# rvp-group/srrg2_slam_interfaces

Measured on AMD Instinct MI355X. Metric: icp_iterations_per_sec, higher is better.
Workload: dtype f32; 1 GPU; C2: SE(3) point-to-plane AlignerSlice, 100000-pt synthetic cloud pair per GPU, 10 ICP iterations per compute(), gated NN 0.25 m + normal gate, Cauchy 0.05; points=100000, alignments_total=1, all_success=True, last_status=0, last_num_inliers=99432, parallelism=single GPU

## Files before the change

### srrg2_slam_interfaces_amd/csrc/kernels.hip

```cpp
#include <climits>
#include <cstdlib>
#include <algorithm>

#include "kernels.h"
#include "search_plan.h"

#include <type_traits>

#include "det_math.h"

#include "device_util.h"

namespace {

#define FX_MAGIC 6755399441055744.0
#define FX_MAGIC_BITS 0x4338000000000000ll
__device__ __forceinline__ long long fx_bits(double biased) { return __double_as_longlong(biased) - FX_MAGIC_BITS; }

__device__ __forceinline__ unsigned long long key_min(unsigned long long a, unsigned long long b) {
  double r;
  asm("v_min_f64 %0, %1, %2" : "=v"(r) : "v"(__longlong_as_double((long long) a)), "v"(__longlong_as_double((long long) b)));
  return (unsigned long long) __double_as_longlong(r);
}

// ... 316 lines not shown
      local[threadIdx.x] += v;
    else if (v != 0)
      atomicAdd(reinterpret_cast<unsigned long long*>(partials) +
                  ((size_t) prob * PARTIAL_SLOTS + (block & (PARTIAL_SLOTS - 1))) * ACC_N + threadIdx.x,
                (unsigned long long) v);
  }
}

}

namespace {

struct QEntry {
  int i;
  int r2;
  float best;
  int bidx, bpos;
  float qx, qy, qz;
  float ball2;
  int pad_;
};
static_assert(sizeof(QEntry) == 40, "host reserves 10 words per entry");

__device__ __forceinline__ void finder_transform_of(const float* Sinv, int dim, const float* X, float* T) {
  if (dim == 3) {
    dm::se3_compose(Sinv, X, T);
  } else {
    float t9[9];
    dm::se2_compose(Sinv, X, t9);
    T[0] = t9[0]; T[1] = t9[1]; T[2] = 0.f; T[3] = t9[2];
    T[4] = t9[3]; T[5] = t9[4]; T[6] = 0.f; T[7] = t9[5];
    T[8] = 0.f; T[9] = 0.f; T[10] = 1.f; T[11] = 0.f;
  }
}
__device__ __forceinline__ void load_T(const float* src, float* T) {
#pragma unroll
  for (int i = 0; i < 12; ++i) T[i] = src[i];
}

template <int DIM>
__device__ __forceinline__ void transform_point(const float* T, const float4 p, float& qx, float& qy, float& qz) {
  if constexpr (DIM == 3) {
    qx = ((T[0] * p.x + T[1] * p.y) + T[2] * p.z) + T[3];
    qy = ((T[4] * p.x + T[5] * p.y) + T[6] * p.z) + T[7];
    qz = ((T[8] * p.x + T[9] * p.y) + T[10] * p.z) + T[11];
  } else {
    qx = (T[0] * p.x + T[1] * p.y) + T[3];
    qy = (T[4] * p.x + T[5] * p.y) + T[7];
    qz = 0.f;
  }
}

constexpr int STAGE_CAP = 64;
template <int DIM, int TW, bool STAGE = false>
__device__ __forceinline__ void coop_scan(const GridDev& g, int lane, int* lds_wave, float sqx, float sqy, float sqz,
                                          int scx, int scy, int scz, int sr, float sr2, float& wbest, int& widx,
                                          int& wpos, float& wexcl2, float4* stage = nullptr) {
  constexpr int ROWS_PER_CHUNK = 2 * TW;
  const int lt   = lane & (TW - 1);
  const int team = lane / TW;
  int* flat      = lds_wave + team * (4 * TW + 8);
  int* first     = flat + ROWS_PER_CHUNK + 4;
  const float rr = ball_radius(sr2);
  int x0, x1, y0, y1, z0 = 0, z1 = 0;
  axis_range(sqx, rr, g.ox, g.inv_h, scx - sr, scx + sr, g.nx, x0, x1);
  axis_range(sqy, rr, g.oy, g.inv_h, scy - sr, scy + sr, g.ny, y0, y1);
  if (DIM == 3) axis_range(sqz, rr, g.oz, g.inv_h, scz - sr, scz + sr, g.nz, z0, z1);
  auto row_range = [&](int rrow, int ny_r, int& rs, int& re) {
    const int y = y0 + rrow % ny_r, z = z0 + rrow / ny_r;
    const float ylo = g.oy + (float) y * g.h;
    float dy        = fmaxf(fmaxf(ylo - sqy, sqy - (ylo + g.h)), 0.f);
    dy              = fmaxf(dy - (0.01f * g.h + (fabsf(sqy) + rr) * 2e-6f), 0.f);
    float rem       = rr * rr - dy * dy;
    if (DIM == 3) {
      const float zlo = g.oz + (float) z * g.h;
      float dz        = fmaxf(fmaxf(zlo - sqz, sqz - (zlo + g.h)), 0.f);
      dz              = fmaxf(dz - (0.01f * g.h + (fabsf(sqz) + rr) * 2e-6f), 0.f);
      rem             = rem - dz * dz;
    }
    rs = re = 0;
    if (!(rem < 0.f)) {
      int xa = x0, xb = x1;
      if (rem < 3.0e38f) axis_range(sqx, ball_radius(rem), g.ox, g.inv_h, x0, x1, g.nx, xa, xb);
      if (xa <= xb) {
        const int row = (z * g.ny + y) * g.nx;
        rs = g.cell_start[row + xa];
        re = g.cell_start[row + xb + 1];
      }
    }
  };
  unsigned long long key = NO_KEY;
  float lb2              = INFINITY;
  const bool any = sr >= 0 && x0 <= x1 && y0 <= y1 && z0 <= z1;
  const int ny_r = any ? y1 - y0 + 1 : 1;
  const int rows = any ? ny_r * (z1 - z0 + 1) : 0;
  int max_rows = rows;
  if (TW < 64) {
#pragma unroll
    for (int off = TW; off < 64; off <<= 1) max_rows = max(max_rows, __shfl_xor(max_rows, off));
  }
  [[maybe_unused]] int staged = 0;
  for (int row0 = 0; row0 < max_rows; row0 += ROWS_PER_CHUNK) {
    int sA = 0, eA = 0, sB = 0, eB = 0;
    const int rA = row0 + lt, rB = row0 + TW + lt;
    if (rA < rows) row_range(rA, ny_r, sA, eA);
    if (rB < rows) row_range(rB, ny_r, sB, eB);
    const unsigned long long pk = (unsigned long long) (unsigned) (eA - sA) | ((unsigned long long) (unsigned) (eB - sB) << 32);
    unsigned long long inc = pk;
#pragma unroll
    for (int off = 1; off < TW; off <<= 1) {
      unsigned long long t = __shfl_up(inc, off, TW);
      if (lt >= off) inc += t;
    }
    const unsigned long long tot = __shfl(inc, TW - 1, TW);
    const int totA = (int) (unsigned) tot, totB = (int) (tot >> 32);
    const unsigned long long exc = inc - pk;
    flat[lt]       = (int) (unsigned) exc;
    flat[TW + lt]  = totA + (int) (exc >> 32);
    first[lt]      = sA;
    first[TW + lt] = sB;
    if (lt == 0) flat[ROWS_PER_CHUNK] = totA + totB;
    wave_lds_sync();
    const int total = totA + totB;
    const int share = (total + TW - 1) / TW;
    int t           = lt * share;
    const int tend  = min(t + share, total);
    if (t < tend) {
      int lo = 0, hi = ROWS_PER_CHUNK - 1;
#pragma unroll
      for (int it = 0; it < 7; ++it) {
        if ((1 << it) >= ROWS_PER_CHUNK) break;
        const int mid = (lo + hi + 1) >> 1;
        if (flat[mid] <= t) lo = mid; else hi = mid - 1;
      }
      int r    = lo;
      int next = flat[r + 1];
      while (t < tend) {
        while (t >= next) {
          ++r;
          next = flat[r + 1];
        }
        const int j   = first[r] + (t - flat[r]);
        const int run = min(next, tend) - t;
        if constexpr (STAGE) {
          if (staged + total <= STAGE_CAP)
            for (int c = 0; c < run; ++c) stage[staged + t + c] = g.pts[j + c];
        } else {
          scan_range2<DIM>(g.pts, j, j + run, sqx, sqy, sqz, key, lb2);
        }
        t += run;
      }
    }
    if constexpr (STAGE) staged += total;
    wave_lds_sync();
  }
  if constexpr (STAGE) {
    wbest = INFINITY; widx = staged; wpos = 0; wexcl2 = 0.f;
    return;
  }
  unsigned long long kmin = key;
#pragma unroll
  for (int off = TW / 2; off >= 1; off >>= 1) {
    const unsigned long long o = __shfl_xor(kmin, off);
    kmin = o < kmin ? o : kmin;
  }
  wpos  = 0;
  wbest = __uint_as_float((unsigned) (kmin >> 32));
  widx  = (int) (unsigned) kmin;
  float v = key == kmin ? lb2 : fminf(lb2, __uint_as_float((unsigned) (key >> 32)));
#pragma unroll
  for (int off = TW / 2; off >= 1; off >>= 1) v = fminf(v, __shfl_xor(v, off));
  wexcl2 = fminf(v, fminf(sr2, bound2_of(max(sr, 0), g.h)));
}

namespace {

#ifndef SRRG2_CNL_REDEAL
#define SRRG2_CNL_REDEAL 0
#endif
#ifdef SRRG2_CNL_STATS
__device__ unsigned long long g_cnl_stats[4 * 16];
#define CNL_STAT(k, v)                                                                                   \
  do {                                                                                                   \
    const unsigned long long v_ = (unsigned long long) (v);    \
    if ((threadIdx.x & 63) == 0) atomicAdd(&g_cnl_stats[(stat_it < 3 ? stat_it : 3) * 16 + (k)], v_);    \
  } while (0)
#else
#define CNL_STAT(k, v) do { } while (0)
#endif
constexpr int CNL_POOL = 512;

struct CnlWave {
  uint2 pool[CNL_POOL];
  unsigned long long key[64];
  unsigned b2[64];
  float q[3][64];
};

template <int DIM>
// ... 1204 lines not shown
      float wbest, wexcl2;
      int widx, wpos;
      coop_scan<DIM, 64>(g, lane, wlds[wid].coop, __shfl(qx, src), __shfl(qy, src), __shfl(qz, src), __shfl(cx, src),
                         __shfl(cy, src), __shfl(cz, src), __shfl(r2, src), __shfl(ball2, src), wbest, widx, wpos, wexcl2);
      if (lane == src) excl_wide = sqrtf(wexcl2) * 0.99999f;
      if (lane == src && (wbest < best || (wbest == best && widx < bidx))) {
        best = wbest;
        bidx = widx;
      }
      continue;
    }
    int src[4];
#pragma unroll
    for (int t = 0; t < 4; ++t) {
      src[t] = need ? __ffsll((long long) need) - 1 : -1;
      need &= need - 1;
    }
    const int team = lane >> 4;
    const int mine = team == 0 ? src[0] : (team == 1 ? src[1] : (team == 2 ? src[2] : src[3]));
    const int from = mine >= 0 ? mine : lane;
    float wbest, wexcl2;
    int widx, wpos;
    const int sr_from = __shfl(r2, from);
    coop_scan<DIM, 16>(g, lane, wlds[wid].coop, __shfl(qx, from), __shfl(qy, from), __shfl(qz, from), __shfl(cx, from),
                       __shfl(cy, from), __shfl(cz, from), mine >= 0 ? sr_from : -1, __shfl(ball2, from), wbest, widx, wpos,
                       wexcl2);
#pragma unroll
    for (int t = 0; t < 4; ++t) {
      const float rb = __shfl(wbest, 16 * t), re = __shfl(wexcl2, 16 * t);
      const int ri = __shfl(widx, 16 * t);
      if (lane == src[t]) {
        excl_wide = sqrtf(re) * 0.99999f;
        if (rb < best || (rb == best && ri < bidx)) {
          best = rb;
          bidx = ri;
        }
      }
    }
  }
  if (excl_wide != 0.f || r2 != 0) excl = excl_wide;
  long long acc[ACC_N];
#pragma unroll
  for (int a = 0; a < ACC_N; ++a) acc[a] = 0;
  finish_point<DIM, PLANE>(S, T, rk, thr, kk, scale, inrange, active, gi, oi, p, qx, qy, qz, best, bidx, bpos, excl, skipped,
                           pf, pn, pnm, use_prior && S.use_normal_gate, acc);
  block_reduce_store<NW>(acc, S.partials, prob, tile, nullptr);
}

#ifdef SRRG2_PASS_TIMELINE
#define PASS_TS_WGS 2048
__device__ unsigned long long g_pass_ts[16 * PASS_TS_WGS * 8];
#define PASS_TS_ANY(epoch, k)                       \
  do {                                                                                                 \
    if ((threadIdx.x & 63) == 0 && (epoch) >= 0 && (epoch) < 16 && blockIdx.y < PASS_TS_WGS - 2 && blockIdx.x == 0) \
      g_pass_ts[(((epoch) * PASS_TS_WGS) + blockIdx.y) * 8 + (k)] = wall_clock64();                            \
  } while (0)
#define PASS_TS_W(epoch, k, dep)              \
  do {                                                                                                 \
    if (threadIdx.x == 0 && (epoch) >= 0 && (epoch) < 16 && blockIdx.x == 0) {                         \
      unsigned long long t_ = wall_clock64();                                                          \
      if ((dep) != (dep)) t_ = 0;         \
      g_pass_ts[(((epoch) * PASS_TS_WGS) + 0) * 8 + (k)] = t_;                                                  \
    }                                                                                                  \
  } while (0)
#define PASS_TS(epoch, k)                                                                              \
  do {                                                                                                 \
    if (threadIdx.x == 0 && (epoch) >= 0 && (epoch) < 16 && blockIdx.y < PASS_TS_WGS - 2 && blockIdx.x == 0)       \
      g_pass_ts[(((epoch) * PASS_TS_WGS) + blockIdx.y) * 8 + (k)] = wall_clock64();                            \
  } while (0)
#else
#define PASS_TS(epoch, k) do { } while (0)
#define PASS_TS_ANY(epoch, k) do { } while (0)
#define PASS_TS_W(epoch, k, dep) do { } while (0)
#endif
namespace {

__device__ float robust_weight(int kind, float thr, float chi, bool& kernelized);
template <bool PAIRS = false, bool GIVEN = true>
__device__ __forceinline__ int slice_exponent(const CtlParams& C, const SliceCtl& s, int prob, int nm, const float* T,
                                              int* kh_out = nullptr);
template <bool ONLY_INLINE, bool PAIRS = false>
__device__ __forceinline__ void init_problem_thread0(const CtlParams& C, int prob, const ProblemDev* probs_host, ProblemDev* probs,
                                                     ProblemState* states, const float* guesses_host, int tsize,
                                                     const InitInline& inl, unsigned (*init_gran)[PUB_SLICE_GRANULES]);

__device__ __forceinline__ double rl_d(double v, int k) {
  const int lo = __builtin_amdgcn_readlane(__double2loint(v), k);
  const int hi = __builtin_amdgcn_readlane(__double2hiint(v), k);
  return __hiloint2double(hi, lo);
}
__device__ __forceinline__ long long rl_ll(long long v, int k) {
  const int lo = __builtin_amdgcn_readlane((int) (unsigned) v, k);
  const int hi = __builtin_amdgcn_readlane((int) (unsigned) ((unsigned long long) v >> 32), k);
  return (long long) (((unsigned long long) (unsigned) hi << 32) | (unsigned) lo);
}
__device__ __forceinline__ float rl_f(float v, int k) { return __int_as_float(__builtin_amdgcn_readlane(__float_as_int(v), k)); }
__device__ __forceinline__ double wave_max_d(double v) {
#pragma unroll
  for (int off = 32; off >= 1; off >>= 1) {
    const double o = __shfl_xor(v, off);
    v              = o > v ? o : v;
  }
  return v;
}
__device__ __forceinline__ double wave_min_d(double v) {
#pragma unroll
  for (int off = 32; off >= 1; off >>= 1) {
    const double o = __shfl_xor(v, off);
    v              = o < v ? o : v;
  }
  return v;
}

__device__ __forceinline__ unsigned long long pub_load(const unsigned long long* p) {
  return __hip_atomic_load(p, __ATOMIC_RELAXED, __HIP_MEMORY_SCOPE_AGENT);
}
__device__ __forceinline__ void pub_store(unsigned long long* p, unsigned long long v) {
  __hip_atomic_store(p, v, __ATOMIC_RELAXED, __HIP_MEMORY_SCOPE_AGENT);
}

// ... 481 lines not shown

struct PassView {
  float T[12], Tprev[12];
  int kexp;
  bool stop, phase1, prior;
};

__device__ __forceinline__ void pass_view_legacy(const SliceDev& S, const ProblemState* __restrict__ st, PassView& v) {
#pragma unroll
  for (int i = 0; i < 12; ++i) v.T[i] = st->Tf[S.slice_idx][i];
#pragma unroll
  for (int i = 0; i < 12; ++i) v.Tprev[i] = st->Tfprev[S.slice_idx][i];
  v.kexp   = st->kexp[S.slice_idx];
  v.stop   = st->done || st->finished;
  v.phase1 = st->phase == 1;
  v.prior  = st->nstats > 0 || st->phase == 1;
}

#ifndef SRRG2_FUSED_POLL_LIMIT
#define SRRG2_FUSED_POLL_LIMIT 64
#endif
#ifdef SRRG2_FUSED_STALL
__device__ unsigned long long g_fused_fallbacks;
extern "C" int srrg2_amd_debug_fused_fallbacks(unsigned long long* out, int reset) {
  if (out && hipMemcpyFromSymbol(out, HIP_SYMBOL(g_fused_fallbacks), sizeof(unsigned long long)) != hipSuccess) return -1;
  if (reset) {
    const unsigned long long zero = 0;
    if (hipMemcpyToSymbol(HIP_SYMBOL(g_fused_fallbacks), &zero, sizeof(zero)) != hipSuccess) return -1;
  }
  return 0;
}
#define FUSED_STALL()                                                              \
  do {                                                                             \
    for (int stall_i = 0; stall_i < (SRRG2_FUSED_STALL); ++stall_i) __builtin_amdgcn_s_sleep(127); \
  } while (0)
#define FUSED_FALLBACK_COUNT()                                                     \
  do {                                                                             \
    if ((threadIdx.x & 63) == 0) atomicAdd(&g_fused_fallbacks, 1ull);              \
  } while (0)
__device__ unsigned long long g_stage_counts[6];
extern "C" int srrg2_amd_debug_staged_neighbours(unsigned long long* out6, int reset) {
  if (out6 && hipMemcpyFromSymbol(out6, HIP_SYMBOL(g_stage_counts), 6 * sizeof(unsigned long long)) != hipSuccess) return -1;
  if (reset) {
    const unsigned long long zero[6] = {0, 0, 0, 0, 0, 0};
    if (hipMemcpyToSymbol(HIP_SYMBOL(g_stage_counts), zero, sizeof(zero)) != hipSuccess) return -1;
  }
  return 0;
}
#define STAGE_COUNT(k, n)                                   \
  do {                                                                             \
    const unsigned long long n_ = (unsigned long long) (n);                        \
    if ((threadIdx.x & 63) == 0 && n_) atomicAdd(&g_stage_counts[k], n_);          \
  } while (0)
#else
#define FUSED_STALL() do { } while (0)
#define FUSED_FALLBACK_COUNT() do { } while (0)
#ifdef SRRG2_PASS_TIMELINE
#define STAGE_COUNT(k, n)                                                                                        \
  do {                                                                                                           \
    const unsigned long long n_ = (unsigned long long) (n);                                                      \
    if ((threadIdx.x & 63) == 0 && n_ && S.fc.epoch >= 0 && S.fc.epoch < 16 && blockIdx.x == 0)                  \
      atomicAdd(&g_pass_ts[((size_t) S.fc.epoch * PASS_TS_WGS + PASS_TS_WGS - 2) * 8 + (k)], n_);                \
  } while (0)
#else
#define STAGE_COUNT(k, n) do { } while (0)
#endif
#endif
#ifndef STAGE_THIN_A
#define STAGE_THIN_A 2.0f
#endif
#ifndef STAGE_THIN_B
#define STAGE_THIN_B 1e-5f
#endif

template <int DIM, bool PRIORS = false>
__device__ __forceinline__ void fused_control_if_due(const SliceDev& S, ProblemState* __restrict__ states, int prob) {
  if (blockIdx.y != 0 || threadIdx.x >= 64) return;
  const unsigned long long g[1] = {
    pub_load(S.fc.pub + ((size_t) prob * SRRG2_MAX_SLICES + S.slice_idx) * PUB_SLICE_GRANULES + (threadIdx.x & 63))};
  if (!__all((unsigned) (g[0] >> 32) == (unsigned) S.fc.epoch)) {
    FUSED_STALL();
    wave_control<DIM == 3 ? 6 : 3, 1, true, PRIORS>(&S, 1, states, prob, g);
  }
  PASS_TS(S.fc.epoch, 1);
}

struct NoStaging {};
template <int DIM, bool PRIORS = false, class WhileWaiting = NoStaging>
__device__ __forceinline__ void pass_view_fused(const SliceDev& S, ProblemState* __restrict__ states, int prob, PassView& v,
                                                WhileWaiting while_waiting = WhileWaiting{}) {
  constexpr bool STAGING = !std::is_same<WhileWaiting, NoStaging>::value;
  __shared__ unsigned rec_lds[PUB_SLICE_GRANULES];
  [[maybe_unused]] __shared__ unsigned stale_lds[STAGING ? 25 : 1];
  const int lane = threadIdx.x & 63;
  [[maybe_unused]] unsigned long long g_first = 0;
  if constexpr (STAGING) {
    if (threadIdx.x < 64) {
      const unsigned long long* rec = S.fc.pub + ((size_t) prob * SRRG2_MAX_SLICES + S.slice_idx) * PUB_SLICE_GRANULES + lane;
      const bool late = (int) (blockIdx.y * gridDim.x + blockIdx.x) >= S.fc.first_round;
      g_first         = late ? *rec : pub_load(rec);
      const bool whole_prev = __all((unsigned) (g_first >> 32) == (unsigned) (S.fc.epoch - 1));
      if (lane < 24) stale_lds[lane] = (unsigned) g_first;
      if (lane == 24) stale_lds[24] = whole_prev ? 1u : 0u;
    }
    __syncthreads();
    while_waiting(stale_lds);
  }
  if (threadIdx.x < 64) {
    const unsigned long long* rec = S.fc.pub + ((size_t) prob * SRRG2_MAX_SLICES + S.slice_idx) * PUB_SLICE_GRANULES + lane;
    const bool late      = (int) (blockIdx.y * gridDim.x + blockIdx.x) >= S.fc.first_round;
    unsigned long long g;
    if constexpr (STAGING) g = g_first; else g = late ? *rec : pub_load(rec);
    if (!__all((unsigned) (g >> 32) == (unsigned) S.fc.epoch)) {
      const unsigned* ep = S.fc.pub_epoch + ((size_t) prob * PUB_EPOCH_REPLICAS + (blockIdx.y & (PUB_EPOCH_REPLICAS - 1))) * PUB_EPOCH_STRIDE;
      int spins = 0;
      for (;;) {
        if ((int) __hip_atomic_load(ep, __ATOMIC_RELAXED, __HIP_MEMORY_SCOPE_AGENT) >= S.fc.epoch) {
          g = pub_load(rec);
// ... 457 lines not shown
      }
    }
#pragma unroll
    for (int r = 0; r < ROWS; ++r) {
      J[r][0] = m[r][0];
      J[r][1] = m[r][1];
      J[r][2] = m[r][1] * p.x - m[r][0] * p.y;
    }
  }
}

}

template <int DIM, bool PLANE, int PPT, bool GATHER, int FUSED>
__device__ __forceinline__ void icp_step_fast_body(const SliceDev& S, const ProblemDev* __restrict__ probs,
                                                   ProblemState* __restrict__ states) {
  constexpr int D    = DIM == 3 ? 6 : 3;
  constexpr int ROWS = PLANE ? 1 : DIM;
  const int prob     = (FUSED ? blockIdx.x : blockIdx.y) + S.prob0;
  const int tile     = FUSED ? (int) blockIdx.y : (int) blockIdx.x;
  const ProblemState* st = &states[prob];
  PassView pv;
  if constexpr (!FUSED) {
    pass_view_legacy(S, st, pv);
    if (pv.stop) return;
  } else {
    PASS_TS(S.fc.epoch, 0);
    fused_control_if_due<DIM, FUSED == 2>(S, states, prob);
  }
  const ProblemDev pd = probs[prob];
  if (tile * (256 * PPT) >= pd.nm && (!FUSED || tile != 0)) return;
  float T[12], Tprev[12];
  double scale;
  int rk;
  if constexpr (!FUSED) {
    load_T(pv.T, T);
    load_T(pv.Tprev, Tprev);
    scale = dm::pow2(pv.kexp);
    rk    = (pv.phase1 && S.robust_kind != SRRG2_ROBUST_NONE) ? (int) SRRG2_ROBUST_CLAMP : S.robust_kind;
  }
  const float thr    = S.robust_thr;
  const float kk     = S.variable_kind == SRRG2_SE3_QUAT_RIGHT ? 2.f : 1.f;
  const GridDev& g   = S.grid;
  const float gfar   = g.gate2_ext;
  const int rfar     = g.rmax;
  const float gate_r = S.gate * 1.000001f;
  const bool ngate   = S.use_normal_gate != 0;
  const bool use_q   = !FUSED && S.queue != nullptr && st->qmode[S.slice_idx] != 0;
  const int lane     = threadIdx.x & 63;
  const int wid      = threadIdx.x >> 6;
  struct StageWave {
    int coop[288];
    float4 cand[4][STAGE_CAP];
  };
  union FastWaveLds {
    CnlWave cnl;
    int coop[288];
    StageWave stage;
  };
  static_assert(sizeof(StageWave) <= sizeof(CnlWave), "the staged candidates live in the idle pool of the list search");
  __shared__ FastWaveLds fast_lds[4];
  int* const coop_lds_w = fast_lds[wid].coop;

  auto linearize = [&](auto first, long long (&acc)[ACC_N], bool valid, const float4 pk, const float4 fk, const float4 nk,
                       const float4 nmk, float qx, float qy, float qz, float best) {
    bool found = valid && __float_as_int(fk.w) != NO_MATCH && best <= g.gate2;
    if (ngate) {
      float dot;
      if constexpr (DIM == 3) {
        const float rx = (T[0] * nmk.x + T[1] * nmk.y) + T[2] * nmk.z;
        const float ry = (T[4] * nmk.x + T[5] * nmk.y) + T[6] * nmk.z;
        const float rz = (T[8] * nmk.x + T[9] * nmk.y) + T[10] * nmk.z;
        dot            = (nk.x * rx + nk.y * ry) + nk.z * rz;
      } else {
        const float rx = T[0] * nmk.x + T[1] * nmk.y;
        const float ry = T[4] * nmk.x + T[5] * nmk.y;
        dot            = nk.x * rx + nk.y * ry;
      }
      found = found && dot > S.normal_cos;
    }
    float J[ROWS][D], e[ROWS];
    point_rows<DIM, PLANE>(T, kk, pk, qx, qy, qz, fk, nk, J, e);
    (void) factor_accumulate_flat<D, ROWS, decltype(first)::value>(J, e, found, rk, thr, scale, acc);
  };

  long long acc[ACC_N];

  float4 p[PPT], pf[PPT], pnm[PPT], pn[PPT];
  float pm[PPT];
  int gi_[PPT];
  bool inr[PPT];
#pragma unroll
  for (int k = 0; k < PPT; ++k) {
    const int i = (tile * PPT + k) * 256 + (int) threadIdx.x;
    inr[k]      = i < pd.nm;
    gi_[k]      = pd.moff + (inr[k] ? i : 0);
    int ppos    = -1;
    p[k]        = S.mpts[gi_[k]];
    pm[k]       = S.prev_m[gi_[k]];
    pf[k]       = make_float4(0.f, 0.f, 0.f, __int_as_float(NO_MATCH));
    pn[k]       = make_float4(0.f, 0.f, 0.f, 0.f);
    pnm[k]      = make_float4(0.f, 0.f, 0.f, 0.f);
    if (GATHER) {
      ppos = S.prev_pos[gi_[k]];
    } else {
      pf[k] = S.prev_f[gi_[k]];
      if (PLANE || ngate) pn[k] = S.prev_n[gi_[k]];
    }
    if (ngate) pnm[k] = S.mnrm[gi_[k]];
    if (GATHER && ppos >= 0 && ppos < g.n) {
      pf[k] = g.pts[ppos];
      if (PLANE || ngate) pn[k] = g.nrm[ppos];
    }
  }
  constexpr bool STAGE = PPT == 1 && FUSED == 1 && !GATHER;
  [[maybe_unused]] unsigned long long st_mask = 0;
  [[maybe_unused]] int st_n = 0;
  [[maybe_unused]] float st_R2 = 0.f;
  [[maybe_unused]] float Tst[12];
  [[maybe_unused]] auto stage_thin = [&](const unsigned* stale) {
    if (!__builtin_amdgcn_readfirstlane((int) stale[24])) return;
    float Tpp[12];
#pragma unroll
    for (int i = 0; i < 12; ++i) Tst[i] = __int_as_float(__builtin_amdgcn_readfirstlane((int) stale[i]));
#pragma unroll
    for (int i = 0; i < 12; ++i) Tpp[i] = __int_as_float(__builtin_amdgcn_readfirstlane((int) stale[12 + i]));
    float ax, ay, az, bx, by, bz;
    transform_point<DIM>(Tst, p[0], ax, ay, az);
    transform_point<DIM>(Tpp, p[0], bx, by, bz);
    const float ex = ax - bx, ey = ay - by, ez = az - bz;
    const float dlp = __builtin_amdgcn_sqrtf((ex * ex + ey * ey) + ez * ez);
    unsigned long long k0 = NO_KEY;
    test_candidate<DIM>(pf[0], ax, ay, az, true, k0);
    const float d0 = __builtin_amdgcn_sqrtf(key_best(k0));
    const float rr = (d0 + PAD_MIN * g.h) * 1.00001f;
    const float R2 = fminf(rr * rr, gfar);
    const bool thin = inr[0] && finite3(p[0].x, p[0].y, p[0].z) && __float_as_int(pf[0].w) != NO_MATCH &&
                      R2 <= bound2_of(2, g.h) && pm[0] * 0.99999f - d0 * 1.00001f < STAGE_THIN_A * dlp + STAGE_THIN_B * g.h;
    unsigned long long m = __ballot(thin);
    const int nthin      = __popcll(m);
    if (nthin == 0) return;
    if (nthin > 4) {
      STAGE_COUNT(5, 1);
      return;
    }
    st_mask = m;
    st_R2   = R2;
    int src[4];
#pragma unroll
    for (int t = 0; t < 4; ++t) {
      src[t] = m ? __ffsll((long long) m) - 1 : -1;
      m &= m - 1;
    }
    const int team = lane >> 4;
    const int mine = team == 0 ? src[0] : (team == 1 ? src[1] : (team == 2 ? src[2] : src[3]));
    const int from = mine >= 0 ? mine : lane;
    const float sqx = __shfl(ax, from), sqy = __shfl(ay, from), sqz = __shfl(az, from), sball = __shfl(R2, from);
    const int scx = cell_coord(sqx, g.ox, g.inv_h), scy = cell_coord(sqy, g.oy, g.inv_h);
    const int scz = DIM == 3 ? cell_coord(sqz, g.oz, g.inv_h) : 0;
    float wbest, wexcl2;
    int wpos, count;
    coop_scan<DIM, 16, true>(g, lane, fast_lds[wid].stage.coop, sqx, sqy, sqz, scx, scy, scz, mine >= 0 ? 2 : -1, sball, wbest,
                             count, wpos, wexcl2, fast_lds[wid].stage.cand[team]);
    st_n = mine >= 0 ? count : 0;
    STAGE_COUNT(0, nthin);
    PASS_TS_ANY(S.fc.epoch, 5);
  };
  if constexpr (FUSED) {
    if constexpr (STAGE)
      pass_view_fused<DIM, false>(S, states, prob, pv, stage_thin);
    else
      pass_view_fused<DIM, FUSED == 2>(S, states, prob, pv);
    if (pv.stop || tile * (256 * PPT) >= pd.nm) return;
    load_T(pv.T, T);
    load_T(pv.Tprev, Tprev);
    scale = dm::pow2(pv.kexp);
    rk    = (pv.phase1 && S.robust_kind != SRRG2_ROBUST_NONE) ? (int) SRRG2_ROBUST_CLAMP : S.robust_kind;
  }

  float open_ball2[PPT];
  bool any_open = false;
  auto search_open = [&](float (&sbest)[PPT], int (&sidx)[PPT], float (&sexcl)[PPT], int (&spos)[PPT]) {
  #pragma unroll
    for (int k = 0; k < PPT; ++k) {
      sbest[k] = INFINITY; sexcl[k] = 0.f; sidx[k] = NO_MATCH; spos[k] = 0;
      bool open = open_ball2[k] >= 0.f;
      if (!__ballot(open)) continue;
      float qx = 0.f, qy = 0.f, qz = 0.f;
      if (open) transform_point<DIM>(T, p[k], qx, qy, qz);
      if constexpr (STAGE) {
        const unsigned long long due = st_mask & __ballot(open);
        STAGE_COUNT(4, __popcll(__ballot(open) & ~st_mask));
        if (due) {
          int src[4];
          unsigned long long m = st_mask;
#pragma unroll
          for (int t = 0; t < 4; ++t) {
            src[t] = m ? __ffsll((long long) m) - 1 : -1;
            m &= m - 1;
          }
          const int team = lane >> 4, lt = lane & 15;
          const int mine = team == 0 ? src[0] : (team == 1 ? src[1] : (team == 2 ? src[2] : src[3]));
          const int from = mine >= 0 ? mine : lane;
          const float sqx = __shfl(qx, from), sqy = __shfl(qy, from), sqz = __shfl(qz, from);
          const bool work = mine >= 0 && ((due >> (mine & 63)) & 1ull) && st_n <= STAGE_CAP;
          unsigned long long key = NO_KEY;
          float lb2 = INFINITY;
          if (work) {
            const float4* cand = fast_lds[wid].stage.cand[team];
            for (int c = lt; c < st_n; c += 16) test_candidate2<DIM>(cand[c], sqx, sqy, sqz, true, key, lb2);
          }
          unsigned long long kmin = key;
#pragma unroll
          for (int off = 8; off >= 1; off >>= 1) {
            const unsigned long long o = __shfl_xor(kmin, off);
            kmin = o < kmin ? o : kmin;
          }
          float v = key == kmin ? lb2 : fminf(lb2, key_best(key));
#pragma unroll
          for (int off = 8; off >= 1; off >>= 1) v = fminf(v, __shfl_xor(v, off));
          bool decided = false, overflow = false;
#pragma unroll
          for (int t = 0; t < 4; ++t) {
            const unsigned long long rk_ = __shfl(kmin, 16 * t);
            const float rv = __shfl(v, 16 * t);
            const int rn   = __shfl(st_n, 16 * t);
            if (lane == src[t] && open) {
              float ax, ay, az;
              transform_point<DIM>(Tst, p[k], ax, ay, az);
              const float ex = qx - ax, ey = qy - ay, ez = qz - az;
              const float dls = sqrtf((ex * ex + ey * ey) + ez * ez);
              const float rin = sqrtf(st_R2) * 0.99999f - dls * 1.00001f;
              overflow = rn > STAGE_CAP;
              if (!overflow && key_idx(rk_) != NO_MATCH && sqrtf(key_best(rk_)) * 1.00001f < rin) {
                sbest[k] = key_best(rk_);
                sidx[k]  = key_idx(rk_);
                sexcl[k] = sqrtf(fminf(rv, rin * rin)) * 0.99999f;
                decided  = true;
              }
            }
          }
          STAGE_COUNT(1, __popcll(__ballot(decided)));
          STAGE_COUNT(2, __popcll(__ballot(overflow)));
          STAGE_COUNT(3, __popcll(due) - __popcll(__ballot(decided || overflow)));
          open = open && !decided;
          if (!__ballot(open)) continue;
        }
      }
      if (g.list_R > 0 && __popcll(__ballot(open)) > 4) {
        unsigned long long skey;
        float sb2, sL;
        cnl_search<DIM, 1>(g, *g.lists, fast_lds[wid].cnl, lane, open, qx, qy, qz, open_ball2[k], gfar, skey, sb2, sL);
        if (open) {
          sbest[k] = key_best(skey);
          sidx[k]  = key_idx(skey);
          sexcl[k] = sqrtf(fminf(sb2, fminf(sL, g.gate2_ext))) * 0.99999f;
        }
        continue;
      }
      bool open_k = open;
      if constexpr (PPT == 1) {
        if (!(g.list_R > 0) && __popcll(__ballot(open)) > 4) {
          unsigned long long lkey = NO_KEY;
          float lb2 = INFINITY, lc2 = INFINITY;
          if (open)
            scan_radius1<DIM>(g, qx, qy, qz, cell_coord(qx, g.ox, g.inv_h), cell_coord(qy, g.oy, g.inv_h),
                              DIM == 3 ? cell_coord(qz, g.oz, g.inv_h) : 0, open_ball2[k], lkey, lb2, lc2);
          const float b2_1 = bound2_of(1, g.h);
          if (open && key_idx(lkey) != NO_MATCH && key_best(lkey) <= gfar && key_best(lkey) <= b2_1) {
            sbest[k] = key_best(lkey);
            sidx[k]  = key_idx(lkey);
            sexcl[k] = sqrtf(fminf(fminf(lb2, lc2), b2_1)) * 0.99999f;
            open_k   = false;
          }
        }
      }
      const int r2 = open_ball2[k] <= bound2_of(2, g.h) ? 2 : max(rfar, 3);
      unsigned long long near = __ballot(open_k && r2 == 2);
      while (near) {
        int src[4];
  #pragma unroll
        for (int t = 0; t < 4; ++t) {
          src[t] = near ? __ffsll((long long) near) - 1 : -1;
          near &= near - 1;
        }
        const int team = lane >> 4;
        const int mine = team == 0 ? src[0] : (team == 1 ? src[1] : (team == 2 ? src[2] : src[3]));
        const int from = mine >= 0 ? mine : lane;
        const float sqx = __shfl(qx, from), sqy = __shfl(qy, from), sqz = __shfl(qz, from), sball = __shfl(open_ball2[k], from);
        const int scx = cell_coord(sqx, g.ox, g.inv_h), scy = cell_coord(sqy, g.oy, g.inv_h);
        const int scz = DIM == 3 ? cell_coord(sqz, g.oz, g.inv_h) : 0;
// ... 34 lines not shown
  };
  constexpr bool defer = PPT == 1 && FUSED;
  float d_qx = 0.f, d_qy = 0.f, d_qz = 0.f, d_best = INFINITY;
  bool d_valid = false;
#pragma unroll
  for (int k = 0; k < PPT; ++k) {
    const bool active = inr[k] && finite3(p[k].x, p[k].y, p[k].z);
    float qx, qy, qz, px, py, pz;
    transform_point<DIM>(T, p[k], qx, qy, qz);
    transform_point<DIM>(Tprev, p[k], px, py, pz);
    const float ex = qx - px, ey = qy - py, ez = qz - pz;
    const float dl   = __builtin_amdgcn_sqrtf((ex * ex + ey * ey) + ez * ez);
    const bool hasp  = __float_as_int(pf[k].w) != NO_MATCH;
    unsigned long long k1 = NO_KEY;
    test_candidate<DIM>(pf[k], qx, qy, qz, true, k1);
    const float best = key_best(k1);
    const float d1   = __builtin_amdgcn_sqrtf(best);
    const float rhs  = pm[k] * 0.99999f;
    const bool ca   = hasp && (d1 * 1.00001f + dl * 1.00001f < rhs);
    const bool cc   = !hasp && pm[k] > 0.f && (gate_r * 1.00001f + dl * 1.00001f < rhs);
    const bool have = active && (ca || cc);
    const float excl = pm[k] * 0.9999999f - dl * 1.00001f;
    const float pad  = fminf(2.f * dl, PAD_CAP * g.h) + PAD_MIN * g.h;
    const float rr   = (d1 + pad) * 1.00001f;
    const float r2box = hasp ? fminf(rr * rr, gfar) : gfar;
    open_ball2[k]     = (active && !have) ? r2box : -1.f;
    any_open |= active && !have;
#ifdef SRRG2_PASS_TIMELINE
    if constexpr (FUSED) {
      if (active && !have && S.fc.epoch >= 0 && S.fc.epoch < 16 && blockIdx.x == 0) {
        unsigned long long* c = &g_pass_ts[((size_t) S.fc.epoch * PASS_TS_WGS + PASS_TS_WGS - 1) * 8];
        const float gap = (pm[k] - d1) / g.h;
        atomicAdd(&c[0], 1ull);
        if (!hasp) atomicAdd(&c[1], 1ull);
        else if (gap < 1e-4f) atomicAdd(&c[2], 1ull);
        else if (gap < 0.0202f) atomicAdd(&c[3], 1ull);
        else atomicAdd(&c[4], 1ull);
        if (dl > 1e-3f * g.h) atomicAdd(&c[5], 1ull);
        if (pm[k] <= 0.f) atomicAdd(&c[6], 1ull);
      }
    }
#endif
    if constexpr (defer) {
      d_qx = qx; d_qy = qy; d_qz = qz; d_best = best; d_valid = have && ca;
    } else if (k == 0) {
      linearize(std::true_type{}, acc, have && ca, p[k], pf[k], pn[k], pnm[k], qx, qy, qz, best);
    } else {
      linearize(std::false_type{}, acc, have && ca, p[k], pf[k], pn[k], pnm[k], qx, qy, qz, best);
    }
    if (have) S.prev_m[gi_[k]] = excl;
  }
  if constexpr (defer) {
    {
      if (__any(any_open)) {
        float sbest[PPT], sexcl[PPT];
        int sidx[PPT], spos[PPT];
        search_open(sbest, sidx, sexcl, spos);
        const bool open = open_ball2[0] >= 0.f;
        const bool same = open && sidx[0] != NO_MATCH && sidx[0] == __float_as_int(pf[0].w);
        if (open && !same) {
          pf[0] = make_float4(0.f, 0.f, 0.f, __int_as_float(NO_MATCH));
          pn[0] = make_float4(0.f, 0.f, 0.f, 0.f);
          if (sidx[0] != NO_MATCH) {
            spos[0] = g.pos_of[sidx[0]];
            pf[0]   = g.pts[spos[0]];
            if (PLANE || ngate) pn[0] = g.nrm[spos[0]];
          }
          S.prev_pos[gi_[0]] = sidx[0] != NO_MATCH ? spos[0] : -1;
          if (!GATHER) {
            S.prev_f[gi_[0]] = pf[0];
            if (PLANE || ngate) S.prev_n[gi_[0]] = pn[0];
          }
        }
        if (open) {
          S.prev_m[gi_[0]] = sexcl[0];
          d_best  = sbest[0];
          d_valid = true;
        }
      }
      linearize(std::true_type{}, acc, d_valid, p[0], pf[0], pn[0], pnm[0], d_qx, d_qy, d_qz, d_best);
      block_reduce_store_biased<4>(acc, S.partials, prob, tile, PPT);
      if constexpr (FUSED) PASS_TS(S.fc.epoch, 3);
      return;
    }
  }
  if (use_q) {
#pragma unroll
    for (int k = 0; k < PPT; ++k) {
      const bool open               = open_ball2[k] >= 0.f;
      const unsigned long long need = __ballot(open);
      if (!need) continue;
      const int r2 = open_ball2[k] <= bound2_of(2, g.h) ? 2 : max(rfar, 3);
      const unsigned long long need_near = __ballot(open && r2 == 2);
      const unsigned long long need_far  = need & ~need_near;
      int base_near = 0, base_far = 0;
      if (lane == 0) {
        if (need_near) base_near = atomicAdd(&S.qcount[2 * prob], __popcll(need_near));
        if (need_far) base_far = atomicAdd(&S.qcount[2 * prob + 1], __popcll(need_far));
      }
      base_near = __shfl(base_near, 0);
      base_far  = __shfl(base_far, 0);
      if (open) {
        const unsigned long long below = (1ull << lane) - 1ull;
        QEntry q;
        q.i = (tile * PPT + k) * 256 + (int) threadIdx.x;
        q.r2 = r2; q.best = INFINITY; q.bidx = NO_MATCH; q.bpos = 0;
        transform_point<DIM>(T, p[k], q.qx, q.qy, q.qz);
        q.ball2 = open_ball2[k]; q.pad_ = 0;
        QEntry* qbase = reinterpret_cast<QEntry*>(S.queue) + pd.moff;
        if (r2 == 2)
          qbase[base_near + __popcll(need_near & below)] = q;
        else
          qbase[pd.nm - 1 - (base_far + __popcll(need_far & below))] = q;
      }
    }
  }
  block_reduce_store_biased<4, 1>(acc, S.partials, prob, tile, PPT);
  if (use_q || !__any(any_open)) {
    block_reduce_store_biased<4, 2>(acc, S.partials, prob, tile, PPT);
    if constexpr (FUSED) PASS_TS(S.fc.epoch, 3);
    return;
  }

  float sbest[PPT], sexcl[PPT];
  int sidx[PPT], spos[PPT];
  search_open(sbest, sidx, sexcl, spos);
  long long acc2[ACC_N];
#pragma unroll
  for (int k = 0; k < PPT; ++k) {
    const bool open = open_ball2[k] >= 0.f;
    float4 fk = make_float4(0.f, 0.f, 0.f, __int_as_float(NO_MATCH)), nk = make_float4(0.f, 0.f, 0.f, 0.f);
    bool same = false;
    if constexpr (PPT == 1) same = open && sidx[k] != NO_MATCH && sidx[k] == __float_as_int(pf[k].w);
    if (same) {
// ... 2227 lines not shown
```

Measured before the change: 65140 iterations/s.

## Add per-query near-candidate fast path and thin-lane fallback in staged NN search

Result: faster. 66310 iterations/s, median of 6 (+1.8%).

```diff
diff --git a/srrg2_slam_interfaces_amd/csrc/kernels.hip b/srrg2_slam_interfaces_amd/csrc/kernels.hip
--- a/srrg2_slam_interfaces_amd/csrc/kernels.hip
+++ b/srrg2_slam_interfaces_amd/csrc/kernels.hip
@@ -392,10 +392,15 @@
 }
 
 constexpr int STAGE_CAP = 64;
+constexpr int STAGE_NEAR = 5;
+struct StageNear {
+  int n[4];
+  float4 f[4][STAGE_NEAR];
+};
 template <int DIM, int TW, bool STAGE = false>
 __device__ __forceinline__ void coop_scan(const GridDev& g, int lane, int* lds_wave, float sqx, float sqy, float sqz,
                                           int scx, int scy, int scz, int sr, float sr2, float& wbest, int& widx,
-                                          int& wpos, float& wexcl2, float4* stage = nullptr) {
+                                          int& wpos, float& wexcl2, float4* stage = nullptr, StageNear* near = nullptr) {
   constexpr int ROWS_PER_CHUNK = 2 * TW;
   const int lt   = lane & (TW - 1);
   const int team = lane / TW;
@@ -484,7 +489,14 @@
         const int run = min(next, tend) - t;
         if constexpr (STAGE) {
           if (staged + total <= STAGE_CAP)
-            for (int c = 0; c < run; ++c) stage[staged + t + c] = g.pts[j + c];
+            for (int c = 0; c < run; ++c) {
+              const float4 f        = g.pts[j + c];
+              stage[staged + t + c] = f;
+              if (!(cand_d2<DIM>(f, sqx, sqy, sqz) > sr2 * 1.000001f)) {
+                const int at = atomicAdd(&near->n[team], 1);
+                if (at < STAGE_NEAR) near->f[team][at] = f;
+              }
+            }
         } else {
           scan_range2<DIM>(g.pts, j, j + run, sqx, sqy, sqz, key, lb2);
         }
@@ -1795,7 +1807,7 @@
 __device__ unsigned long long g_pass_ts[16 * PASS_TS_WGS * 8];
 #define PASS_TS_ANY(epoch, k)                       \
   do {                                                                                                 \
-    if ((threadIdx.x & 63) == 0 && (epoch) >= 0 && (epoch) < 16 && blockIdx.y < PASS_TS_WGS - 2 && blockIdx.x == 0) \
+    if ((threadIdx.x & 63) == 0 && (epoch) >= 0 && (epoch) < 16 && blockIdx.y < PASS_TS_WGS - 3 && blockIdx.x == 0) \
       g_pass_ts[(((epoch) * PASS_TS_WGS) + blockIdx.y) * 8 + (k)] = wall_clock64();                            \
   } while (0)
 #define PASS_TS_W(epoch, k, dep)              \
@@ -1808,7 +1820,7 @@
   } while (0)
 #define PASS_TS(epoch, k)                                                                              \
   do {                                                                                                 \
-    if (threadIdx.x == 0 && (epoch) >= 0 && (epoch) < 16 && blockIdx.y < PASS_TS_WGS - 2 && blockIdx.x == 0)       \
+    if (threadIdx.x == 0 && (epoch) >= 0 && (epoch) < 16 && blockIdx.y < PASS_TS_WGS - 3 && blockIdx.x == 0)       \
       g_pass_ts[(((epoch) * PASS_TS_WGS) + blockIdx.y) * 8 + (k)] = wall_clock64();                            \
   } while (0)
 #else
@@ -2396,6 +2408,20 @@
     const unsigned long long n_ = (unsigned long long) (n);                        \
     if ((threadIdx.x & 63) == 0 && n_) atomicAdd(&g_stage_counts[k], n_);          \
   } while (0)
+__device__ unsigned long long g_stage_winners[5];
+extern "C" int srrg2_amd_debug_staged_winners(unsigned long long* out5, int reset) {
+  if (out5 && hipMemcpyFromSymbol(out5, HIP_SYMBOL(g_stage_winners), 5 * sizeof(unsigned long long)) != hipSuccess) return -1;
+  if (reset) {
+    const unsigned long long zero[5] = {0, 0, 0, 0, 0};
+    if (hipMemcpyToSymbol(HIP_SYMBOL(g_stage_winners), zero, sizeof(zero)) != hipSuccess) return -1;
+  }
+  return 0;
+}
+#define STAGE_WIN(k, n)                                     \
+  do {                                                                             \
+    const unsigned long long n_ = (unsigned long long) (n);                        \
+    if ((threadIdx.x & 63) == 0 && n_) atomicAdd(&g_stage_winners[k], n_);         \
+  } while (0)
 #else
 #define FUSED_STALL() do { } while (0)
 #define FUSED_FALLBACK_COUNT() do { } while (0)
@@ -2406,8 +2432,15 @@
     if ((threadIdx.x & 63) == 0 && n_ && S.fc.epoch >= 0 && S.fc.epoch < 16 && blockIdx.x == 0)                  \
       atomicAdd(&g_pass_ts[((size_t) S.fc.epoch * PASS_TS_WGS + PASS_TS_WGS - 2) * 8 + (k)], n_);                \
   } while (0)
+#define STAGE_WIN(k, n)       \
+  do {                                                                                                           \
+    const unsigned long long n_ = (unsigned long long) (n);                                                      \
+    if ((threadIdx.x & 63) == 0 && n_ && S.fc.epoch >= 0 && S.fc.epoch < 16 && blockIdx.x == 0)                  \
+      atomicAdd(&g_pass_ts[((size_t) S.fc.epoch * PASS_TS_WGS + PASS_TS_WGS - 3) * 8 + (k)], n_);                \
+  } while (0)
 #else
 #define STAGE_COUNT(k, n) do { } while (0)
+#define STAGE_WIN(k, n) do { } while (0)
 #endif
 #endif
 #ifndef STAGE_THIN_A
@@ -2971,6 +3004,7 @@
   struct StageWave {
     int coop[288];
     float4 cand[4][STAGE_CAP];
+    StageNear near;
   };
   union FastWaveLds {
     CnlWave cnl;
@@ -3033,10 +3067,12 @@
     }
   }
   constexpr bool STAGE = PPT == 1 && FUSED == 1 && !GATHER;
+  [[maybe_unused]] int st_near = -1;
   [[maybe_unused]] unsigned long long st_mask = 0;
   [[maybe_unused]] int st_n = 0;
   [[maybe_unused]] float st_R2 = 0.f;
   [[maybe_unused]] float Tst[12];
+  [[maybe_unused]] bool st_dec = false, st_own = false;
   [[maybe_unused]] auto stage_thin = [&](const unsigned* stale) {
     if (!__builtin_amdgcn_readfirstlane((int) stale[24])) return;
     float Tpp[12];
@@ -3057,14 +3093,18 @@
     const bool thin = inr[0] && finite3(p[0].x, p[0].y, p[0].z) && __float_as_int(pf[0].w) != NO_MATCH &&
                       R2 <= bound2_of(2, g.h) && pm[0] * 0.99999f - d0 * 1.00001f < STAGE_THIN_A * dlp + STAGE_THIN_B * g.h;
     unsigned long long m = __ballot(thin);
-    const int nthin      = __popcll(m);
+    int nthin            = __popcll(m);
     if (nthin == 0) return;
     if (nthin > 4) {
       STAGE_COUNT(5, 1);
-      return;
+      m     = __ballot(thin && pm[0] * 0.99999f - d0 * 1.00001f < STAGE_THIN_B * g.h);
+      nthin = __popcll(m);
+      if (nthin == 0 || nthin > 4) return;
+      STAGE_WIN(3, nthin);
     }
     st_mask = m;
     st_R2   = R2;
+    if ((m >> lane) & 1ull) st_near = __popcll(m & ((1ull << lane) - 1ull));
     int src[4];
 #pragma unroll
     for (int t = 0; t < 4; ++t) {
@@ -3079,10 +3119,12 @@
     const int scz = DIM == 3 ? cell_coord(sqz, g.oz, g.inv_h) : 0;
     float wbest, wexcl2;
     int wpos, count;
+    if ((lane & 15) == 0) fast_lds[wid].stage.near.n[team] = 0;
     coop_scan<DIM, 16, true>(g, lane, fast_lds[wid].stage.coop, sqx, sqy, sqz, scx, scy, scz, mine >= 0 ? 2 : -1, sball, wbest,
-                             count, wpos, wexcl2, fast_lds[wid].stage.cand[team]);
+                             count, wpos, wexcl2, fast_lds[wid].stage.cand[team], &fast_lds[wid].stage.near);
     st_n = mine >= 0 ? count : 0;
     STAGE_COUNT(0, nthin);
+    if ((lane & 15) == 0 && count > STAGE_CAP) fast_lds[wid].stage.near.n[team] = STAGE_NEAR + 1;
     PASS_TS_ANY(S.fc.epoch, 5);
   };
   if constexpr (FUSED) {
@@ -3111,51 +3153,76 @@
         const unsigned long long due = st_mask & __ballot(open);
         STAGE_COUNT(4, __popcll(__ballot(open) & ~st_mask));
         if (due) {
-          int src[4];
-          unsigned long long m = st_mask;
-#pragma unroll
-          for (int t = 0; t < 4; ++t) {
-            src[t] = m ? __ffsll((long long) m) - 1 : -1;
-            m &= m - 1;
+          bool decided = false, overflow = false;
+          auto accept = [&](unsigned long long wk, float wv) {
+            float ax, ay, az;
+            transform_point<DIM>(Tst, p[k], ax, ay, az);
+            const float ex = qx - ax, ey = qy - ay, ez = qz - az;
+            const float dls = sqrtf((ex * ex + ey * ey) + ez * ez);
+            const float rin = sqrtf(st_R2) * 0.99999f - dls * 1.00001f;
+            if (key_idx(wk) != NO_MATCH && sqrtf(key_best(wk)) * 1.00001f < rin) {
+              sbest[k] = key_best(wk);
+              sidx[k]  = key_idx(wk);
+              sexcl[k] = sqrtf(fminf(wv, rin * rin)) * 0.99999f;
+              decided  = true;
+              st_dec   = true;
+            }
+          };
+          bool quick = false;
+          if (open && st_near >= 0) {
+            const StageNear& near = fast_lds[wid].stage.near;
+            const int n_near      = near.n[st_near];
+            float4 nf[STAGE_NEAR];
+#pragma unroll
+            for (int i = 0; i < STAGE_NEAR; ++i) nf[i] = near.f[st_near][i];
+            quick = n_near <= STAGE_NEAR;
+            if (quick) {
+              unsigned long long key = NO_KEY;
+              float lb2 = INFINITY;
+#pragma unroll
+              for (int i = 0; i < STAGE_NEAR; ++i) test_candidate2<DIM>(nf[i], qx, qy, qz, i < n_near, key, lb2);
+              accept(key, lb2);
+              st_own = decided;
+            }
           }
-          const int team = lane >> 4, lt = lane & 15;
-          const int mine = team == 0 ? src[0] : (team == 1 ? src[1] : (team == 2 ? src[2] : src[3]));
-          const int from = mine >= 0 ? mine : lane;
-          const float sqx = __shfl(qx, from), sqy = __shfl(qy, from), sqz = __shfl(qz, from);
-          const bool work = mine >= 0 && ((due >> (mine & 63)) & 1ull) && st_n <= STAGE_CAP;
-          unsigned long long key = NO_KEY;
-          float lb2 = INFINITY;
-          if (work) {
-            const float4* cand = fast_lds[wid].stage.cand[team];
-            for (int c = lt; c < st_n; c += 16) test_candidate2<DIM>(cand[c], sqx, sqy, sqz, true, key, lb2);
-          }
-          unsigned long long kmin = key;
-#pragma unroll
-          for (int off = 8; off >= 1; off >>= 1) {
-            const unsigned long long o = __shfl_xor(kmin, off);
-            kmin = o < kmin ? o : kmin;
-          }
-          float v = key == kmin ? lb2 : fminf(lb2, key_best(key));
-#pragma unroll
-          for (int off = 8; off >= 1; off >>= 1) v = fminf(v, __shfl_xor(v, off));
-          bool decided = false, overflow = false;
-#pragma unroll
-          for (int t = 0; t < 4; ++t) {
-            const unsigned long long rk_ = __shfl(kmin, 16 * t);
-            const float rv = __shfl(v, 16 * t);
-            const int rn   = __shfl(st_n, 16 * t);
-            if (lane == src[t] && open) {
-              float ax, ay, az;
-              transform_point<DIM>(Tst, p[k], ax, ay, az);
-              const float ex = qx - ax, ey = qy - ay, ez = qz - az;
-              const float dls = sqrtf((ex * ex + ey * ey) + ez * ez);
-              const float rin = sqrtf(st_R2) * 0.99999f - dls * 1.00001f;
-              overflow = rn > STAGE_CAP;
-              if (!overflow && key_idx(rk_) != NO_MATCH && sqrtf(key_best(rk_)) * 1.00001f < rin) {
-                sbest[k] = key_best(rk_);
-                sidx[k]  = key_idx(rk_);
-                sexcl[k] = sqrtf(fminf(rv, rin * rin)) * 0.99999f;
-                decided  = true;
+          STAGE_WIN(4, __popcll(__ballot(quick && decided)));
+          const unsigned long long due_team = due & ~__ballot(quick);
+          if (due_team) {
+            int src[4];
+            unsigned long long m = st_mask;
+#pragma unroll
+            for (int t = 0; t < 4; ++t) {
+              src[t] = m ? __ffsll((long long) m) - 1 : -1;
+              m &= m - 1;
+            }
+            const int team = lane >> 4, lt = lane & 15;
+            const int mine = team == 0 ? src[0] : (team == 1 ? src[1] : (team == 2 ? src[2] : src[3]));
+            const int from = mine >= 0 ? mine : lane;
+            const float sqx = __shfl(qx, from), sqy = __shfl(qy, from), sqz = __shfl(qz, from);
+            const bool work = mine >= 0 && ((due_team >> (mine & 63)) & 1ull) && st_n <= STAGE_CAP;
+            unsigned long long key = NO_KEY;
+            float lb2 = INFINITY;
+            if (work) {
+              const float4* cand = fast_lds[wid].stage.cand[team];
+              for (int c = lt; c < st_n; c += 16) test_candidate2<DIM>(cand[c], sqx, sqy, sqz, true, key, lb2);
+            }
+            unsigned long long kmin = key;
+#pragma unroll
+            for (int off = 8; off >= 1; off >>= 1) {
+              const unsigned long long o = __shfl_xor(kmin, off);
+              kmin = o < kmin ? o : kmin;
+            }
+            float v = key == kmin ? lb2 : fminf(lb2, key_best(key));
+#pragma unroll
+            for (int off = 8; off >= 1; off >>= 1) v = fminf(v, __shfl_xor(v, off));
+#pragma unroll
+            for (int t = 0; t < 4; ++t) {
+              const unsigned long long rk_ = __shfl(kmin, 16 * t);
+              const float rv = __shfl(v, 16 * t);
+              const int rn   = __shfl(st_n, 16 * t);
+              if (lane == src[t] && open && !quick) {
+                overflow = rn > STAGE_CAP;
+                if (!overflow) accept(rk_, rv);
               }
             }
           }
@@ -3296,10 +3363,12 @@
   }
   if constexpr (defer) {
     {
+      [[maybe_unused]] int stamp_w = 0;
       if (__any(any_open)) {
         float sbest[PPT], sexcl[PPT];
         int sidx[PPT], spos[PPT];
         search_open(sbest, sidx, sexcl, spos);
+        if constexpr (STAGE) PASS_TS_ANY(S.fc.epoch, 4);
         const bool open = open_ball2[0] >= 0.f;
         const bool same = open && sidx[0] != NO_MATCH && sidx[0] == __float_as_int(pf[0].w);
         if (open && !same) {
@@ -3321,9 +3390,18 @@
           d_best  = sbest[0];
           d_valid = true;
         }
+        if constexpr (STAGE) {
+          STAGE_WIN(0, __popcll(__ballot(st_dec && same)));
+          STAGE_WIN(2, __popcll(__ballot(st_dec && !same)));
+          stamp_w = (__ballot(open && !same) ? 1 : 0) | (__ballot(st_own) ? 2 : 0);
+        }
       }
       linearize(std::true_type{}, acc, d_valid, p[0], pf[0], pn[0], pnm[0], d_qx, d_qy, d_qz, d_best);
       block_reduce_store_biased<4>(acc, S.partials, prob, tile, PPT);
+      if constexpr (STAGE) {
+        if (stamp_w & 1) PASS_TS_ANY(S.fc.epoch, 6);
+        if (stamp_w & 2) PASS_TS_ANY(S.fc.epoch, 7);
+      }
       if constexpr (FUSED) PASS_TS(S.fc.epoch, 3);
       return;
     }
```
